# shininglegend/cs420-ray-tracer

Hardware: NVIDIA B200
Metric: Mrays/s (higher is better)
Workload: dtype f32 filter / f64 decide

## Files before the change

### cs420-ray-tracer_b200/csrc/kernels_fast.cuh

```cuda
#ifndef RT_KERNELS_FAST_CUH
#define RT_KERNELS_FAST_CUH

#include "bvh.cuh"
#include "exact_fp64.cuh"
#include "filter_math.cuh"
#include "rt_device.h"

namespace rtf {

using rtx::d3;

#ifndef RT_THREADS
#define RT_THREADS 256
#endif
constexpr int kThreads = RT_THREADS;
constexpr int kWarps = kThreads / 32;
constexpr unsigned kTwoMult = 1, kLpMult = 4;
constexpr int kWTileW = 16, kWTileH = 4;
constexpr int kGroupPairs = 4;
constexpr int kSmemHeader = 2048;
constexpr float kEps = 0.001f;
constexpr unsigned kSign = 0x80000000u;
constexpr unsigned kFull = 0xffffffffu;

struct __align__(16) RayRec {
  double ox, oy, oz, dx, dy, dz;
  unsigned pix;
  float wt;
  float ar, ag, ab;
  unsigned pad;
};

struct FastArgs {
  RtRenderArgs r;
  const unsigned char *tabs;
  int npairs, ngroups;
  int N, L;
  unsigned tstride, gmin_off, perm_off, inv_off, cullA_off, cullB_off;
  unsigned stage_bytes;
  float d64;
  float gS2;
  float g_dtmax;
  double c0[3];
  int wtiles_x, nwtiles;
  unsigned int *tile_counter;
  RayRec *q_out; unsigned int *q_out_count;
  RayRec *q_in; const unsigned int *q_in_count;
  unsigned int *chunk_counter;
  int level;
  int tables_in_smem;
  rtb::BvhView bvh;
  int nbig, big[8];
  unsigned two_mult, lp_mult;
  unsigned queue_cap;
  unsigned int *err;
};

struct Tab {
  const float4 *pairs;
  const float *gmin;
  const int *perm;
  const int *inv;
  const float4 *cullA;
  const float *cullB;
};

__device__ __forceinline__ unsigned fbits(float x) { return __float_as_uint(x); }
__device__ __forceinline__ float f_rd(double x) { return __double2float_rd(x); }
__device__ __forceinline__ float f_ru(double x) { return __double2float_ru(x); }
__device__ __forceinline__ d3 ldc3(const double *p) { return rtx::mk(p[0], p[1], p[2]); }
__device__ __forceinline__ double4 ld_sph64(const double4 *p) {
  const double2 *q = reinterpret_cast<const double2 *>(p);
  double2 a = __ldg(q), b = __ldg(q + 1);
  return make_double4(a.x, a.y, b.x, b.y);
}
__device__ __forceinline__ unsigned long long wsum(unsigned long long v) {
#pragma unroll
  for (int o = 16; o > 0; o >>= 1) v += __shfl_xor_sync(kFull, v, o);
// ... 29 lines not shown
  const float rdv = fmaxf(0.0f, __fmaf_rn(rz, vz, __fmaf_rn(ry, vy, __fmul_rn(rx, vx))));
  const float spec = __fmul_rn(0.5f, shin == 0.0f ? 1.0f : __powf(rdv, shin));
  sr = __fadd_rn(sr, __fmaf_rn(g_frame.light_col[l][0], spec, __fmul_rn(m.x, kd)));
  sg = __fadd_rn(sg, __fmaf_rn(g_frame.light_col[l][1], spec, __fmul_rn(m.y, kd)));
  sb = __fadd_rn(sb, __fmaf_rn(g_frame.light_col[l][2], spec, __fmul_rn(m.z, kd)));
}
__device__ __forceinline__ void write_final(const RtRenderArgs &r, unsigned pix, float cr, float cg, float cb) {
  size_t o = pix;
  if (r.out_remap) {
    const unsigned lr = pix / (unsigned)r.W, x = pix - lr * (unsigned)r.W;
    if (r.out_remap == 2) o = (size_t)rt_local_to_global_row(r.bands, (int)lr) * (size_t)r.W + x;
    else o = (size_t)(lr + (unsigned)r.out_y0) * (size_t)r.out_pitch + x + (unsigned)r.out_x0;
  }
  if (r.fb) { float *f = r.fb + o * 3; f[0] = cr; f[1] = cg; f[2] = cb; }
  else { unsigned char *q = r.rgb + o * 3; q[0] = (unsigned char)quant8(cr); q[1] = (unsigned char)quant8(cg); q[2] = (unsigned char)quant8(cb); }
}
__device__ __forceinline__ int warp_fetch(unsigned int *counter) {
  int v = 0;
  if ((threadIdx.x & 31) == 0) v = (int)atomicAdd(counter, 1u);
  return __shfl_sync(kFull, v, 0);
}

#define RT_PDL_SYNC() do { asm volatile("griddepcontrol.wait;" ::: "memory"); asm volatile("griddepcontrol.launch_dependents;" ::: "memory"); } while (0)

__device__ __forceinline__ void mbar_init(unsigned long long *bar, unsigned count) {
  unsigned a = (unsigned)__cvta_generic_to_shared(bar);
  asm volatile("mbarrier.init.shared::cta.b64 [%0], %1;" ::"r"(a), "r"(count));
  asm volatile("fence.mbarrier_init.release.cluster;" ::: "memory");
}
__device__ __forceinline__ void mbar_expect_tx(unsigned long long *bar, unsigned bytes) {
  unsigned a = (unsigned)__cvta_generic_to_shared(bar);
  asm volatile("mbarrier.arrive.expect_tx.shared::cta.b64 _, [%0], %1;" ::"r"(a), "r"(bytes) : "memory");
}
__device__ __forceinline__ void tma_bulk_g2s(void *dst, const void *src, unsigned bytes, unsigned long long *bar) {
  unsigned d = (unsigned)__cvta_generic_to_shared(dst), b = (unsigned)__cvta_generic_to_shared(bar);
  asm volatile("cp.async.bulk.shared::cluster.global.mbarrier::complete_tx::bytes [%0], [%1], %2, [%3];" ::"r"(d), "l"(src),
               "r"(bytes), "r"(b)
               : "memory");
}
__device__ __forceinline__ void mbar_wait(unsigned long long *bar, unsigned parity) {
  unsigned a = (unsigned)__cvta_generic_to_shared(bar);
  asm volatile(
      "{\n\t.reg .pred p;\n\t"
      "WAIT_%=:\n\t"
      "mbarrier.try_wait.parity.shared::cta.b64 p, [%0], %1;\n\t"
      "@p bra DONE_%=;\n\t"
// ... 1024 lines not shown
  }
  c.closest = c.hits = c.shadow = c.occluded = c.fp64 = c.violations = 0;
  n_fp64 = 0;
}

#ifndef RT_TAIL_THREADS
#define RT_TAIL_THREADS 128
#endif
#ifndef RT_TAIL_CTAS
#define RT_TAIL_CTAS 3
#endif
constexpr int kTailThreads = RT_TAIL_THREADS;
#ifdef RT_TAIL_TRACE
constexpr int kTraceWarps = 4096, kTraceLevels = 6, kTraceStamps = 12;
__device__ unsigned long long g_tail_trace[kTraceWarps * kTraceLevels * kTraceStamps];
#define RT_TT(k, extra) do { const unsigned long long x_ = (unsigned long long)(extra);    \
    if (tt_on && lane == 0 && level - a.level < kTraceLevels) g_tail_trace[(tt_warp * kTraceLevels + (level - a.level)) * kTraceStamps + (k)] = (unsigned long long)clock64() | (x_ << 48); } while (0)
#define RT_TG(k) do { if (tt_on && lane == 0 && level - a.level < kTraceLevels) { unsigned long long t_; asm volatile("mov.u64 %0, %globaltimer;" : "=l"(t_)); g_tail_trace[(tt_warp * kTraceLevels + (level - a.level)) * kTraceStamps + (k)] = t_; } } while (0)
#else
#define RT_TT(k, extra) do { } while (0)
#define RT_TG(k) do { } while (0)
#endif
template <bool kSmem, bool kBvh>
__global__ void __launch_bounds__(kTailThreads, RT_TAIL_CTAS) k_bounce(const FastArgs a) {
  extern __shared__ __align__(128) unsigned char smem[];
  const unsigned char *tabs = a.tabs + a.tstride;
  if (kSmem) { stage_tables(smem, tabs, a.stage_bytes); tabs = smem + kSmemHeader; }
  RT_PDL_SYNC();
  const unsigned nq = *a.q_in_count;
  if (nq == 0u) return;
  const WarpBuf wb = warp_buf(smem + kSmemHeader + ((a.stage_bytes + 127u) & ~127u));
  const float4 *gen = reinterpret_cast<const float4 *>(tabs + (size_t)a.L * a.tstride);
  const int lane = threadIdx.x & 31;
  const int depth = a.r.max_depth, L = a.L;
  Counters cnt = {0, 0, 0, 0, 0, 0};
  int n_fp64 = 0;
  unsigned c_cand = 0, c_walks = 0;
  RayRec *qin = a.q_in;
  const unsigned nwarps = gridDim.x * (unsigned)(kTailThreads / 32);
  const unsigned per = min(32u, max(4u, (nq + nwarps - 1u) / nwarps));
#ifdef RT_TAIL_TRACE
  const unsigned tt_warp = blockIdx.x * (unsigned)(kTailThreads / 32) + (threadIdx.x >> 5);
  bool tt_on = tt_warp < (unsigned)kTraceWarps;
#endif
  for (;;) {
    const int chunk = warp_fetch(a.chunk_counter);
    if ((unsigned)chunk * per >= nq) break;
// ... 171 lines not shown
          } else {
            final_ = true;
          }
        } else {
          add_scaled(cr, cg, cb, wt, sr, sg, sb);
          final_ = true;
        }
      }
      if (live[0] && final_) write_final(a.r, pix, cr, cg, cb);
      if (a.r.counters) {
        flush_counters(a, cnt, n_fp64, level);
        if (lane == 0 && c_walks) { atomicAdd(&a.r.counters[RT_CNT_CAND], (unsigned long long)c_cand); atomicAdd(&a.r.counters[RT_CNT_WALKS], (unsigned long long)c_walks); }
        c_cand = c_walks = 0;
      }
      RT_TT(5, __popc(__ballot_sync(kFull, cont))); RT_TG(7);
      live[0] = cont;
      if (!__any_sync(kFull, cont)) break;
    }
#ifdef RT_TAIL_TRACE
    tt_on = false;
#endif
  }
}

}
#endif
```

### cs420-ray-tracer_b200/csrc/kernels_wave.cuh

```cuda
#ifndef RT_KERNELS_WAVE_CUH
#define RT_KERNELS_WAVE_CUH

#include <type_traits>

#include "kernels_fast.cuh"

#ifndef RT_SHADOW_CTAS
#define RT_SHADOW_CTAS 2
#endif
#ifndef RT_CLOSEST_CTAS
#define RT_CLOSEST_CTAS 2
#endif
#ifndef RT_CLOSEST0_CTAS
#define RT_CLOSEST0_CTAS RT_CLOSEST_CTAS
#endif
namespace rtf {

struct __align__(16) HitRec {
  double px, py, pz;
  float nx, ny, nz;
  float vx, vy, vz;
  int idx;
  unsigned pix;
  unsigned src;
  float wt, ar, ag, ab;
  unsigned pad;
};
__device__ __forceinline__ double hit_d0x(const HitRec &h) { return __hiloint2double(__float_as_int(h.vz), __float_as_int(h.vy)); }
__device__ __forceinline__ double hit_d0y(const HitRec &h) { return __hiloint2double(__float_as_int(h.wt), (int)h.src); }
__device__ __forceinline__ double hit_d0z(const HitRec &h) { return __hiloint2double(__float_as_int(h.ag), __float_as_int(h.ar)); }
__device__ __forceinline__ unsigned hit_ray_rank(const HitRec &h) { return __float_as_uint(h.vx); }
static_assert(sizeof(HitRec) == 80, "hit record layout");

struct WaveArgs {
  FastArgs f;
  HitRec *hits; unsigned int *hit_count;
  unsigned int *hit_n;
  unsigned hit_cap;
  unsigned char *occ;
  int occ_bits;
  unsigned int *work_counter;
  Best *cand;
  unsigned int *work_counter2;
  unsigned int *tile_ray;
};

enum { CTL_TILE = 0, CTL_ERR = 5, CTL_TAIL = 8, CTL_SHADOW = 48, CTL_SHADE = 88, CTL_CLOSEST = 128, CTL_HITS = 168, CTL_RAYS = 208,
       CTL_WORDS = 256 };

__device__ __forceinline__ void hit_block(const WaveArgs &w, unsigned m0, unsigned m1, unsigned (&slot)[2]) {
  const int lane = threadIdx.x & 31;
  const unsigned n = (unsigned)(__popc(m0) + __popc(m1));
  unsigned base = 0;
  if (n != 0u) {
    if (lane == 0) {
      base = atomicAdd(w.hit_count, 64u);
      if (base + 64u > w.hit_cap) { atomicOr(w.f.err, (unsigned)RT_GUARD_HIT_BLOCKS); base = 0u; }
      w.hit_n[base >> 6] = n;
    }
    base = __shfl_sync(kFull, base, 0);
  }
  const unsigned lt = (1u << lane) - 1u;
  slot[0] = base + (unsigned)__popc(m0 & lt);
  slot[1] = base + (unsigned)__popc(m0) + (unsigned)__popc(m1 & lt);
}

__device__ __noinline__ void flush_counts(unsigned long long *counters, int level, unsigned closest, unsigned hits, unsigned shadow,
                                          unsigned occluded, unsigned fp64, unsigned violations, unsigned long long n_spheres,
                                          unsigned cand = 0, unsigned walks = 0, unsigned fallbacks = 0) {
  unsigned v[6] = {closest, hits, shadow, occluded, fp64, violations};
#pragma unroll
// ... 195 lines not shown
        c_closest++; c_fp64 += best[r].nfp64;
        if (best[r].idx >= 0) {
          HitRec *rec = w.hits + hslot[r];
          const int hi = finish_hit(a, best[r], src[r], pix[r], 0u, 1.0f, 0.f, 0.f, 0.f, rec, &c_viol, &c_fp64);
          hit = hi >= 0;
          if (!hit) { rec->idx = -1; rec->pix = pix[r]; }
          else cont[r] = depth > 1 && __ldg(&a.r.matx[hi]).y > 0.5f;
          if (a.r.hit_idx) a.r.hit_idx[(size_t)pix[r] * depth] = hit ? rec->idx : -1;
        } else if (a.r.hit_idx) a.r.hit_idx[(size_t)pix[r] * depth] = -1;
      }
      c_hits += hit;
      const Rgb skyc = sky_colour(dy[r]);
      const bool sky = live[r] && !hit;
      if (kBytes) {
        unsigned char *q = s_rgb + (((lane >> 4) * 2 + r) * kWTileW + (lane & 15)) * 3;
        q[0] = (unsigned char)quant8(sky ? skyc.r : 0.f);
        q[1] = (unsigned char)quant8(sky ? skyc.g : 0.f);
        q[2] = (unsigned char)quant8(sky ? skyc.b : 0.f);
      } else if (sky) {
        write_final(a.r, pix[r], skyc.r, skyc.g, skyc.b);
      }
    }
    {
      const unsigned k0 = __ballot_sync(kFull, cont[0]), k1 = __ballot_sync(kFull, cont[1]), lt = (1u << lane) - 1u;
      if (cont[0]) w.hits[hslot[0]].vx = __uint_as_float((unsigned)__popc(k0 & lt));
      if (cont[1]) w.hits[hslot[1]].vx = __uint_as_float((unsigned)(__popc(k0) + __popc(k1 & lt)));
      if (lane == 0 && tile_ok) w.tile_ray[tile] = (unsigned)(__popc(k0) + __popc(k1));
    }
    if (!kBytes) continue;
    __syncwarp();
    if (!tile_ok || deferred) { __syncwarp(); continue; }
    if (tx0 + kWTileW <= W && (W & 15) == 0) {
      if (lane < kWTileH * 3) {
        const int ty = lane / 3, seg = lane % 3;
        if (ty0 + ty < rows) {
          const size_t orow = kFrame ? (size_t)rt_local_to_global_row(a.r.bands, ty0 + ty) : (size_t)(ty0 + ty);
          *reinterpret_cast<uint4 *>(a.r.rgb + (orow * W + tx0) * 3 + seg * 16) =
              *reinterpret_cast<const uint4 *>(s_rgb + ty * kWTileW * 3 + seg * 16);
        }
      }
    } else {
#pragma unroll
      for (int r = 0; r < 2; r++) {
        if (x < W && lr[r] < rows) {
          const unsigned char *q = s_rgb + (((lane >> 4) * 2 + r) * kWTileW + (lane & 15)) * 3;
          unsigned char *o = a.r.rgb + (kFrame ? ((size_t)j[r] * W + x) : (size_t)pix[r]) * 3;
          o[0] = q[0]; o[1] = q[1]; o[2] = q[2];
        }
      }
    }
    __syncwarp();
  }
  if (a.r.counters) flush_counts(a.r.counters, 0, c_closest, c_hits, 0, 0, c_fp64, c_viol, (unsigned long long)a.N, c_cand, c_walks, c_fall);
}
template <int kMode>
__global__ void __launch_bounds__(kThreads, RT_CLOSEST0_CTAS) k_closest0(const WaveArgs w) {
  extern __shared__ __align__(128) unsigned char smem[];
  const FastArgs &a = w.f;
  const unsigned char *tabs = a.tabs;
  if (kMode == kTabSmem) { stage_tables(smem, a.tabs, a.stage_bytes); tabs = smem + kSmemHeader; }
  if (kMode == kTabStream) ring_init(smem);
  RT_PDL_SYNC();
  closest0_body<kMode>(w, smem, tabs, smem + kSmemHeader + (kMode == kTabBvh ? 0u : ((a.stage_bytes + 127u) & ~127u)));
}

template <bool kBvh, bool kCull = false>
__device__ __forceinline__ void closest1_body(const WaveArgs &w, const float4 *gen, unsigned char *smem) {
  const FastArgs &a = w.f;
  const unsigned nq = __ldcg(a.q_in_count);
  if (nq == 0u) return;
  const int lane = threadIdx.x & 31, depth = a.r.max_depth, level = a.level;
  unsigned c_closest = 0, c_hits = 0, c_fp64 = 0, c_viol = 0, c_cand = 0, c_walks = 0;
  const RayRec *qin = a.q_in;
  static_assert(kGenIds * 2 <= kWTileH * kWTileW * 3, "survivor list in the header's per-warp staging area");
  unsigned short *ids = kCull ? reinterpret_cast<unsigned short *>(smem + 64 + (threadIdx.x >> 5) * (kWTileH * kWTileW * 3)) : nullptr;
  const bool two = nq >= gridDim.x * (unsigned)kWarps * 64u * a.two_mult;
  const unsigned per = two ? 64u : 32u;
  for (;;) {
    const int chunk = warp_fetch(w.work_counter);
    if ((unsigned)chunk * per >= nq) break;
    bool live[2];
    unsigned qi[2], pix[2];
    float ox[2], oy[2], oz[2], dx[2], dy[2], dz[2], wt[2], cr[2], cg[2], cb[2];
#pragma unroll
    for (int r = 0; r < 2; r++) {
// ... 404 lines not shown
        }
      }
    }
  }
  if (a.r.counters) flush_counts(a.r.counters, 99, 0, 0, 0, 0, c_fp64, 0, 0);
}

#ifndef RT_SHADE_CTAS
#define RT_SHADE_CTAS 4
#endif
#ifndef RT_SHADE_UNROLL
#define RT_SHADE_UNROLL 1
#endif
constexpr int kShadeUnroll = RT_SHADE_UNROLL;
__device__ __forceinline__ void prefetch_l1(const void *p) { asm volatile("prefetch.global.L1 [%0];" ::"l"(p)); }
__device__ __forceinline__ void queue_put(const WaveArgs &w, unsigned pos, const RayRec &rec) {
  if (pos < w.f.queue_cap) w.f.q_out[pos] = rec;
  else atomicOr(w.f.err, (unsigned)RT_GUARD_RAY_QUEUE);
}

__device__ __forceinline__ void shade_body(const WaveArgs &w) {
  const FastArgs &a = w.f;
  const int level = a.level;
  const bool ordered = level == 0;
  const unsigned nh = __ldcg(w.hit_count);
  if (nh == 0u) return;
  const int lane = threadIdx.x & 31, L = a.L;
  unsigned c_shadow = 0, c_occ = 0;
  const unsigned G = gridDim.x * (unsigned)kWarps;
  if (ordered && tile_path(a)) {
    __shared__ __align__(16) unsigned char s_tiles[kWarps][kWTileH * kWTileW * 3];
    unsigned char *s_tile = s_tiles[threadIdx.x >> 5];
    const unsigned W = (unsigned)a.r.W, rows = (unsigned)a.r.bands.local_rows;
    const bool frame = a.r.out_remap == 2;
    for (unsigned blk = blockIdx.x * (unsigned)kWarps + (threadIdx.x >> 5); blk * 64u < nh; blk += G) {
      {
        const unsigned bn = blk + G;
        if (bn * 64u < nh) {
          const unsigned char *q = reinterpret_cast<const unsigned char *>(w.hits + bn * 64u) + lane * 128;
          prefetch_l1(q);
          if (lane < 8) prefetch_l1(q + 32 * 128);
          if (lane == 0) prefetch_l1(w.hit_n + bn);
          if (!w.occ_bits && lane < L) prefetch_l1(w.occ + (size_t)lane * w.hit_cap + bn * 64u);
        }
      }
      const unsigned nslots = w.hit_n[blk];
      const unsigned pix0 = w.hits[blk * 64u].pix;
      const unsigned ty0 = (pix0 / W) & ~(unsigned)(kWTileH - 1), tx0 = (pix0 % W) & ~(unsigned)(kWTileW - 1);
      const bool whole = ty0 + kWTileH <= rows;
      const unsigned qbase = w.tile_ray[(ty0 / kWTileH) * (unsigned)a.wtiles_x + tx0 / kWTileW];
      if (whole) {
#pragma unroll
        for (int r = 0; r < 2; r++) {
          const unsigned ly = (unsigned)(lane >> 4) * 2u + (unsigned)r, lx = (unsigned)lane & 15u;
          float fx, fz;
          const unsigned c = sky_rgb8(camera_dir_y(a, (int)(tx0 + lx), rt_local_to_global_row(a.r.bands, (int)(ty0 + ly)), fx, fz));
          unsigned char *q = s_tile + (ly * kWTileW + lx) * 3;
          q[0] = (unsigned char)c; q[1] = (unsigned char)(c >> 8); q[2] = (unsigned char)(c >> 16);
        }
      }
      __syncwarp();
#pragma unroll kShadeUnroll
      for (int half = 0; half < 2; half++) {
        const unsigned h = blk * 64u + (unsigned)half * 32u + lane;
        const bool live = (h & 63u) < nslots && w.hits[h].idx >= 0;
        bool cont = false;
        RayRec rec;
        unsigned rank = 0;
        if (live) {
          const HitRec hr = w.hits[h];
          unsigned long long occm = hr.pad;
          if (!w.occ_bits) {
            occm = 0ull;
            for (int l = 0; l < L; l++)
              if (w.occ[(size_t)l * w.hit_cap + h]) occm |= 1ull << l;
          }
          c_shadow += (unsigned)L; c_occ += (unsigned)__popcll(occm);
          const unsigned y = hr.pix / W, x = hr.pix - y * W;
          cont = shade_one(w, level, hr, occm, rec, whole ? s_tile + ((y - ty0) * kWTileW + (x - tx0)) * 3 : nullptr);
          rank = hit_ray_rank(hr);
        }
        if (cont) queue_put(w, qbase + rank, rec);
      }
      __syncwarp();
      if (whole && lane < kWTileH * 3) {
        const unsigned ty = (unsigned)lane / 3u, sg = (unsigned)lane % 3u;
        const size_t orow = frame ? (size_t)rt_local_to_global_row(a.r.bands, (int)(ty0 + ty)) : (size_t)(ty0 + ty);
        *reinterpret_cast<uint4 *>(a.r.rgb + (orow * W + tx0) * 3 + sg * 16) = *reinterpret_cast<const uint4 *>(s_tile + lane * 16);
      }
      __syncwarp();
    }
    if (a.r.counters) flush_counts(a.r.counters, 99, 0, 0, c_shadow, c_occ, 0, 0, (unsigned long long)a.N);
    return;
  }
  for (unsigned chunk = blockIdx.x * (unsigned)kWarps + (threadIdx.x >> 5); chunk * 32u < nh; chunk += G) {
    const unsigned h = chunk * 32u + lane;
    {
      const unsigned hn = h + G * 32u;
      if (hn < nh) {
        const unsigned char *q = reinterpret_cast<const unsigned char *>(w.hits + hn);
        prefetch_l1(q); prefetch_l1(q + 64);
        if (lane == 0) prefetch_l1(w.hit_n + (hn >> 6));
        if (!w.occ_bits && lane < L) prefetch_l1(w.occ + (size_t)lane * w.hit_cap + hn);
      }
    }
    const bool live = (h & 63u) < w.hit_n[h >> 6] && w.hits[h].idx >= 0;
    bool cont = false;
    RayRec rec;
    unsigned qpos = 0;
    if (live) {
      const HitRec hr = w.hits[h];
      unsigned long long occm = hr.pad;
      if (!w.occ_bits) {
        occm = 0ull;
        for (int l = 0; l < L; l++)
          if (w.occ[(size_t)l * w.hit_cap + h]) occm |= 1ull << l;
      }
      c_shadow += (unsigned)L; c_occ += (unsigned)__popcll(occm);
      cont = shade_one(w, level, hr, occm, rec);
      if (ordered && cont) {
        const unsigned y = hr.pix / (unsigned)a.r.W, x = hr.pix - y * (unsigned)a.r.W;
        qpos = w.tile_ray[(y / kWTileH) * (unsigned)a.wtiles_x + x / kWTileW] + hit_ray_rank(hr);
      }
    }
    if (ordered) { if (cont) queue_put(w, qpos, rec); }
    else queue_push(cont, rec, a.q_out, a.q_out_count, a.queue_cap, a.err);
  }
  if (a.r.counters) flush_counts(a.r.counters, 99, 0, 0, c_shadow, c_occ, 0, 0, (unsigned long long)a.N);
}
__global__ void __launch_bounds__(kThreads, RT_SHADE_CTAS) k_shade(const WaveArgs w) {
  RT_PDL_SYNC();
  shade_body(w);
}

}
#endif
```

### cs420-ray-tracer_b200/csrc/rt_kernels.cu

```cuda
#include "rt_kernels.h"

#include <algorithm>
#include <cmath>
#include <cstring>
#include <map>
#include <mutex>
#include <thread>
#include <tuple>
#include <vector>

__constant__ RtFrameConst g_frame;

#include "kernels_exact.cuh"
#include "kernels_fast.cuh"
#include "kernels_wave.cuh"

cudaError_t rtk_set_frame_const(const RtFrameConst *host_const, cudaStream_t stream) {
  return cudaMemcpyToSymbolAsync(g_frame, host_const, sizeof(RtFrameConst), 0, cudaMemcpyHostToDevice, stream);
}

int rtk_launch_exact(const RtRenderArgs &args, cudaStream_t stream) {
  dim3 block(128);
  dim3 grid((args.W + 31) / 32, (args.bands.local_rows + 3) / 4);
  rtk::k_exact<<<grid, block, 0, stream>>>(args);
// ... 538 lines not shown
    cudaFree(fs->tabs); fs->tabs = nullptr; fs->tabs_cap = 0;
    if (fs->h_stage) cudaFreeHost(fs->h_stage);
    fs->h_stage = nullptr; fs->h_stage_cap = 0;
    fs->sph64 = fs->mat = fs->matx = nullptr;
    cudaFree(fs->bvh_nodes_buf); cudaFree(fs->bvh_scratch); cudaFree(fs->raw_dev);
    fs->bvh_nodes_buf = fs->bvh_scratch = nullptr; fs->bvh_nodes_cap = fs->bvh_scratch_cap = 0;
    fs->raw_dev = nullptr; fs->raw_cap = 0;
  }
  fs->bvh_nodes = fs->bvh_leaves = nullptr; fs->bvh_nleaf = 0;
}

int rtk_fast_last_error(const RtFastWork *w, unsigned int *word) {
  *word = 0;
  if (!w->last_err) return 0;
  RTK_TRY(cudaMemcpy(word, w->last_err, sizeof(unsigned int), cudaMemcpyDeviceToHost));
  return 0;
}

void rtk_fast_free_work(RtFastWork *w) {
  cudaFree(w->queue[0]); cudaFree(w->queue[1]); cudaFree(w->ctl); cudaFree(w->hits); cudaFree(w->occ); cudaFree(w->hit_n); cudaFree(w->cand);
  w->last_err = nullptr;
  w->cand = nullptr; w->cand_cap = 0;
  cudaFree(w->tile_ray); w->tile_ray = nullptr; w->tile_cap = 0;
  if (w->h_fb) { cudaFreeHost(w->h_fb); cudaEventDestroy(w->fb_event); }
  w->h_fb = nullptr; w->fb_pending = 0; w->fb_levels = 0;
  w->queue[0] = w->queue[1] = nullptr; w->ctl = nullptr; w->hits = nullptr; w->occ = nullptr; w->hit_n = nullptr;
  w->queue_cap = w->hit_cap = w->occ_bytes = 0;
}

namespace {
template <typename K>
int resident_grid(K kernel, size_t smem, int num_sms, int threads = rtf::kThreads) {
  static std::mutex mu;
  static std::map<std::tuple<const void *, size_t, int>, int> cache;
  const auto key = std::make_tuple((const void *)kernel, smem, threads);
  std::lock_guard<std::mutex> lk(mu);
  auto it = cache.find(key);
  if (it == cache.end()) {
    int nb = 0;
    if (cudaOccupancyMaxActiveBlocksPerMultiprocessor(&nb, kernel, threads, smem) != cudaSuccess || nb < 1) nb = 1;
    it = cache.emplace(key, nb).first;
  }
  return std::max(1, it->second * num_sms);
}
thread_local cudaError_t g_launch_err = cudaSuccess;
template <typename K, typename A>
void launch(K kernel, int grid, int block, size_t smem, cudaStream_t stream, bool pdl, const A &arg) {
  cudaLaunchConfig_t cfg;
  memset(&cfg, 0, sizeof(cfg));
  cfg.gridDim = dim3((unsigned)grid); cfg.blockDim = dim3((unsigned)block); cfg.dynamicSmemBytes = smem; cfg.stream = stream;
  cudaLaunchAttribute at[1];
  at[0].id = cudaLaunchAttributeProgrammaticStreamSerialization;
  at[0].val.programmaticStreamSerializationAllowed = 1;
  cfg.attrs = at; cfg.numAttrs = pdl ? 1u : 0u;
  const cudaError_t e = cudaLaunchKernelEx(&cfg, kernel, arg);
  if (e != cudaSuccess && g_launch_err == cudaSuccess) g_launch_err = e;
}
inline size_t bvh_smem() { return rtf::kSmemHeader + rtf::kWarps * (size_t)(rtf::kWarpBufBytes + rtf::kBundleBufBytes); }
inline size_t staged_smem(size_t bytes) { return rtf::kSmemHeader + ((bytes + 127) & ~(size_t)127) + rtf::kWarps * (size_t)rtf::kWarpBufBytes; }
using rtf::CTL_TILE; using rtf::CTL_TAIL; using rtf::CTL_SHADOW; using rtf::CTL_SHADE; using rtf::CTL_CLOSEST; using rtf::CTL_HITS; using rtf::CTL_RAYS;
}

int rtk_launch_fast(const RtRenderArgs &args, const RtFastScene *fs, RtFastWork *w, cudaStream_t stream,
                    const cudaEvent_t *marks) {
  const size_t npix = (size_t)args.W * args.bands.local_rows;
  if (!w->ctl) RTK_TRY(cudaMalloc(&w->ctl, kCtlWords * sizeof(unsigned int)));
  const size_t hit_cap = ((size_t)((args.W + rtf::kWTileW - 1) / rtf::kWTileW) * ((args.bands.local_rows + rtf::kWTileH - 1) / rtf::kWTileH) + 2) * 64 +
                         (size_t)w->num_sms * 4 * rtf::kWarps * 128 * (size_t)rtf::kTwoMult;
  if (w->hit_cap < hit_cap || w->occ_bytes < hit_cap * (size_t)(fs->L > 0 ? fs->L : 1) || (args.max_depth > 1 && w->queue_cap < npix)) {
    RTK_TRY(cudaStreamSynchronize(stream));
    cudaFree(w->queue[0]); cudaFree(w->queue[1]); cudaFree(w->hits); cudaFree(w->occ); cudaFree(w->hit_n);
    w->queue[0] = w->queue[1] = nullptr; w->hits = nullptr; w->occ = nullptr; w->hit_n = nullptr; w->queue_cap = w->hit_cap = w->occ_bytes = 0;
    RTK_TRY(cudaMalloc(&w->hits, hit_cap * sizeof(rtf::HitRec)));
    RTK_TRY(cudaMalloc(&w->hit_n, (hit_cap / 64) * sizeof(unsigned int)));
    w->occ_bytes = hit_cap * (size_t)(fs->L > 0 ? fs->L : 1);
    RTK_TRY(cudaMalloc(&w->occ, w->occ_bytes));
    w->hit_cap = hit_cap;
    if (args.max_depth > 1) {
      RTK_TRY(cudaMalloc(&w->queue[0], npix * sizeof(rtf::RayRec)));
      RTK_TRY(cudaMalloc(&w->queue[1], npix * sizeof(rtf::RayRec)));
      w->queue_cap = npix;
    }

  }
  if (fs->bvh_nodes && args.max_depth > 1 && w->cand_cap < npix) {
    RTK_TRY(cudaStreamSynchronize(stream));
    cudaFree(w->cand); w->cand = nullptr; w->cand_cap = 0;
    RTK_TRY(cudaMalloc(&w->cand, npix * sizeof(rtf::Best)));
    w->cand_cap = npix;
  }
  const size_t ntiles = (size_t)((args.W + rtf::kWTileW - 1) / rtf::kWTileW) * ((args.bands.local_rows + rtf::kWTileH - 1) / rtf::kWTileH);
  const size_t tile_cap = (ntiles + 4 * rtf::kThreads - 1) / (4 * rtf::kThreads) * (4 * rtf::kThreads);
  if (w->tile_cap < tile_cap) {
    RTK_TRY(cudaStreamSynchronize(stream));
    cudaFree(w->tile_ray); w->tile_ray = nullptr; w->tile_cap = 0;
    RTK_TRY(cudaMalloc(&w->tile_ray, tile_cap * sizeof(unsigned int)));
    w->tile_cap = tile_cap;
  }
  RTK_TRY(cudaMemsetAsync(w->ctl, 0, kCtlWords * sizeof(unsigned int), stream));
  if (args.max_depth <= 0 && !args.fb && !args.out_remap) RTK_TRY(cudaMemsetAsync(args.rgb, 0, npix * 3, stream));

  g_launch_err = cudaSuccess;
  rtf::WaveArgs wa;
  memset(&wa, 0, sizeof(wa));
  rtf::FastArgs &a = wa.f;
  a.r = args;
  a.tabs = (const unsigned char *)fs->tabs;
  a.npairs = fs->npairs; a.ngroups = fs->ngroups; a.N = fs->N; a.L = fs->L;
  a.tstride = fs->tstride; a.gmin_off = fs->gmin_off; a.perm_off = fs->perm_off; a.inv_off = fs->inv_off;
  a.cullA_off = fs->cullA_off; a.cullB_off = fs->cullB_off;
  a.d64 = fs->d64; a.gS2 = fs->gS2; a.g_dtmax = fs->g_dtmax;
  for (int k = 0; k < 3; k++) a.c0[k] = fs->c0[k];
  a.wtiles_x = (args.W + rtf::kWTileW - 1) / rtf::kWTileW;
  a.nwtiles = a.wtiles_x * ((args.bands.local_rows + rtf::kWTileH - 1) / rtf::kWTileH);
  a.tile_counter = w->ctl + CTL_TILE;
  a.two_mult = rtf::kTwoMult; a.lp_mult = rtf::kLpMult;
  a.queue_cap = (unsigned)w->queue_cap; a.err = w->ctl + rtf::CTL_ERR;
  w->last_err = a.err;
  wa.hits = (rtf::HitRec *)w->hits; wa.hit_cap = (unsigned)hit_cap;
  wa.occ = w->occ; wa.hit_n = w->hit_n; wa.tile_ray = w->tile_ray;
  wa.occ_bits = fs->L <= 32;
  const size_t pairs_bytes = (size_t)fs->npairs * 32;
  const size_t light_bytes = (size_t)fs->L * fs->tstride;
  const bool cam_smem = fs->tstride <= kMaxSmemTables, light_smem = light_bytes <= kMaxSmemTables;
  const bool gen_smem = pairs_bytes <= kMaxSmemTables, in_smem = fs->bytes_bounce <= kMaxSmemTables;
  a.tables_in_smem = in_smem;
  const bool bvh = fs->bvh_nodes != nullptr;
  a.bvh.nodes = (const rtb::BvhNode *)fs->bvh_nodes;
  a.nbig = fs->nbig;
  for (int k = 0; k < 8; k++) a.big[k] = fs->big[k];
  const size_t stream_smem = rtf::kSmemHeader + 2 * (size_t)rtf::kTileBytes;
  int launches = 0;
  const bool pdl = marks == nullptr;

  int wave_levels = w->wave_levels > 0 ? w->wave_levels : (fs->bvh_nodes ? RT_MAX_LEVELS_INTERNAL : (npix >= 750000 ? 2 : 1));
  const unsigned long long fb_key = fs->generation * 1000003ull + (unsigned long long)npix * 131ull + (unsigned long long)args.max_depth;
  const bool fb_auto = w->wave_levels <= 0 && !fs->bvh_nodes && args.max_depth > 1;
  if (fb_auto) {
    if (!w->h_fb) {
      RTK_TRY(cudaHostAlloc(&w->h_fb, 34 * sizeof(unsigned int), cudaHostAllocDefault));
      RTK_TRY(cudaEventCreateWithFlags(&w->fb_event, cudaEventDisableTiming));
    }
    const cudaError_t fbq = w->fb_pending ? cudaEventQuery(w->fb_event) : cudaErrorNotReady;
    if (fbq != cudaSuccess) cudaGetLastError();
    if (w->fb_pending && fbq == cudaSuccess) {
      constexpr unsigned kWaveMinRays = 60000u;
      int lv = 1;
      while (lv < 33 && w->h_fb[lv] >= kWaveMinRays) lv++;
      w->fb_levels = lv; w->fb_key = w->fb_pending_key; w->fb_pending = 0;
    }
    if (w->fb_levels > 0 && w->fb_key == fb_key) wave_levels = w->fb_levels;
  }
  for (int level = 0; level < args.max_depth && level < wave_levels; level++) {
    a.level = level;
    wa.hit_count = w->ctl + CTL_HITS + level;
    if (level == 0) {
      a.stage_bytes = fs->tstride;
      const size_t smem = cam_smem ? staged_smem(a.stage_bytes) : stream_smem;
      const int cta_tiles = (a.nwtiles + rtf::kWarps - 1) / rtf::kWarps;
      if (bvh) { int g = resident_grid(rtf::k_closest0<rtf::kTabBvh>, bvh_smem(), w->num_sms); launch(rtf::k_closest0<rtf::kTabBvh>, g < cta_tiles ? g : cta_tiles, rtf::kThreads, bvh_smem(), stream, false, wa); }
      else if (cam_smem) { int g = resident_grid(rtf::k_closest0<rtf::kTabSmem>, smem, w->num_sms); launch(rtf::k_closest0<rtf::kTabSmem>, g < cta_tiles ? g : cta_tiles, rtf::kThreads, smem, stream, false, wa); }
      else { int g = resident_grid(rtf::k_closest0<rtf::kTabStream>, smem, w->num_sms); launch(rtf::k_closest0<rtf::kTabStream>, g < cta_tiles ? g : cta_tiles, rtf::kThreads, smem, stream, false, wa); }
    } else {
      a.q_in = (rtf::RayRec *)w->queue[(level - 1) & 1];
      a.q_in_count = w->ctl + CTL_RAYS + level;
      wa.work_counter = w->ctl + CTL_CLOSEST + level;
      a.stage_bytes = (unsigned)pairs_bytes;
      const size_t smem = rtf::kSmemHeader + (gen_smem ? a.stage_bytes : 0);
      if (bvh) {
        wa.cand = (rtf::Best *)w->cand;
        wa.work_counter2 = w->ctl + CTL_TAIL + level;
        launch(rtf::k_closest1_dyn, resident_grid(rtf::k_closest1_dyn, 0, w->num_sms), rtf::kThreads, 0, stream, pdl, wa);
        launches++;
        launch(rtf::k_closest1<false, true>, resident_grid(rtf::k_closest1<false, true>, rtf::kSmemHeader, w->num_sms), rtf::kThreads, rtf::kSmemHeader, stream, pdl, wa);
      }
      else if (gen_smem) launch(rtf::k_closest1<true, false>, resident_grid(rtf::k_closest1<true, false>, smem, w->num_sms), rtf::kThreads, smem, stream, pdl, wa);
      else launch(rtf::k_closest1<false, false>, resident_grid(rtf::k_closest1<false, false>, smem, w->num_sms), rtf::kThreads, smem, stream, pdl, wa);
    }
    launches++;
    if (level == 0 && marks) RTK_TRY(cudaEventRecord(marks[0], stream));
    a.q_out = (rtf::RayRec *)w->queue[level & 1];
    a.q_out_count = w->ctl + CTL_RAYS + level + 1;
    if (fs->L > 0 || level == 0) {
      wa.work_counter = w->ctl + CTL_SHADOW + level;
      a.stage_bytes = (unsigned)light_bytes;
      const size_t smem = light_smem ? staged_smem(a.stage_bytes) : stream_smem;
      if (bvh && level > 0) launch(rtf::k_shadow_dyn, resident_grid(rtf::k_shadow_dyn, 0, w->num_sms), rtf::kThreads, 0, stream, pdl, wa);
      else if (bvh) launch(rtf::k_shadow<rtf::kTabBvh>, resident_grid(rtf::k_shadow<rtf::kTabBvh>, bvh_smem(), w->num_sms), rtf::kThreads, bvh_smem(), stream, pdl, wa);
      else if (light_smem) launch(rtf::k_shadow<rtf::kTabSmem>, resident_grid(rtf::k_shadow<rtf::kTabSmem>, smem, w->num_sms), rtf::kThreads, smem, stream, pdl, wa);
      else launch(rtf::k_shadow<rtf::kTabStream>, resident_grid(rtf::k_shadow<rtf::kTabStream>, smem, w->num_sms), rtf::kThreads, smem, stream, pdl, wa);
      launches++;
    }
    if (level == 0 && marks) RTK_TRY(cudaEventRecord(marks[1], stream));
    wa.work_counter = w->ctl + CTL_SHADE + level;
    launch(rtf::k_shade, resident_grid(rtf::k_shade, 0, w->num_sms), rtf::kThreads, 0, stream, pdl, wa);
    launches++;
    if (level == 0 && marks) RTK_TRY(cudaEventRecord(marks[2], stream));
  }
  if (args.max_depth > wave_levels) {
    const int level = wave_levels;
    a.level = level;
    a.q_in = (rtf::RayRec *)w->queue[(level - 1) & 1];
    a.q_in_count = w->ctl + CTL_RAYS + level;
    a.q_out = (rtf::RayRec *)w->queue[level & 1];
    a.q_out_count = w->ctl + CTL_RAYS + level + 1;
    a.chunk_counter = w->ctl + CTL_TAIL + level;
    a.stage_bytes = (unsigned)fs->bytes_bounce;
    const size_t smem = in_smem ? staged_smem(fs->bytes_bounce) : rtf::kSmemHeader;
    if (bvh) launch(rtf::k_bounce<false, true>, resident_grid(rtf::k_bounce<false, true>, rtf::kSmemHeader, w->num_sms, rtf::kTailThreads), rtf::kTailThreads, rtf::kSmemHeader, stream, pdl, a);
    else if (in_smem) launch(rtf::k_bounce<true, false>, resident_grid(rtf::k_bounce<true, false>, smem, w->num_sms, rtf::kTailThreads), rtf::kTailThreads, smem, stream, pdl, a);
    else launch(rtf::k_bounce<false, false>, resident_grid(rtf::k_bounce<false, false>, smem, w->num_sms, rtf::kTailThreads), rtf::kTailThreads, smem, stream, pdl, a);
    launches++;
  }
  if (fb_auto && !w->fb_pending) {
    RTK_TRY(cudaMemcpyAsync(w->h_fb, w->ctl + CTL_RAYS, 34 * sizeof(unsigned int), cudaMemcpyDeviceToHost, stream));
    RTK_TRY(cudaEventRecord(w->fb_event, stream));
    w->fb_pending = 1; w->fb_pending_key = fb_key;
  }
  cudaError_t e = cudaGetLastError();
  if (g_launch_err != cudaSuccess) e = g_launch_err;
  return e == cudaSuccess ? launches : -(int)e;
}

__global__ void k_peer_signal(volatile unsigned int *flag, unsigned int value) {
  __threadfence_system();
  *flag = value;
  __threadfence_system();
}
__global__ void k_peer_wait(volatile unsigned int *flags, int n, unsigned int value, unsigned int *err) {
  const int k = threadIdx.x;
  if (k >= n) return;
  unsigned long long t0, t1;
  asm volatile("mov.u64 %0, %globaltimer;" : "=l"(t0));
  while ((int)(flags[k] - value) < 0) {
    asm volatile("mov.u64 %0, %globaltimer;" : "=l"(t1));
    if (t1 - t0 > 2000000000ULL) { atomicExch(err, 1u + (unsigned)k); break; }
    __nanosleep(200);
  }
  __threadfence_system();
}
int rtk_peer_signal(unsigned int *flag, unsigned int value, cudaStream_t stream) {
  k_peer_signal<<<1, 1, 0, stream>>>(flag, value);
  cudaError_t e = cudaGetLastError();
  return e == cudaSuccess ? 1 : -(int)e;
// ... 84 lines not shown
```

### cs420-ray-tracer_b200/csrc/rt_kernels.h

```cpp
#ifndef RT_KERNELS_H
#define RT_KERNELS_H

#include <cuda_runtime.h>

#include "rt_device.h"

cudaError_t rtk_set_frame_const(const RtFrameConst *host_const, cudaStream_t stream);

int rtk_launch_exact(const RtRenderArgs &args, cudaStream_t stream);

struct RtFastScene {
  int N, L, npairs, ngroups;
  void *tabs;
  size_t tabs_cap;
  void *sph64, *mat, *matx;
  void *h_stage; size_t h_stage_cap;
  void *raw_dev; size_t raw_cap;
  unsigned tstride;
  unsigned gmin_off, perm_off, inv_off, cullA_off, cullB_off;
  size_t bytes_primary;
  size_t bytes_bounce;
  float d64;
  float gS2;
  float g_dtmax;
  unsigned long long generation;
  double c0[3];
  void *bvh_nodes, *bvh_leaves;
  void *bvh_nodes_buf, *bvh_scratch;
  size_t bvh_nodes_cap, bvh_scratch_cap;
  int bvh_nleaf;
  int nbig, big[8];
  double bvh_build_ms;
  double sabs_scene;
  double delta64;
  int lookup_only, device_build;
  void *geo;
  void *cam_scratch; size_t cam_scratch_cap;
};
struct RtFastWork {
  int num_sms;
  int wave_levels;
  unsigned int *h_fb;
  cudaEvent_t fb_event;
  int fb_pending, fb_levels;
  unsigned long long fb_key, fb_pending_key;
  void *queue[2];
  size_t queue_cap;
  unsigned int *ctl;
  unsigned int *last_err;
  void *hits;
  unsigned int *hit_n;
  void *cand;
  size_t cand_cap;
  unsigned char *occ;
  size_t hit_cap, occ_bytes;
  unsigned int *tile_ray;
  size_t tile_cap;
};
int rtk_fast_init(int device);
int rtk_fast_build_scene(RtFastScene *fs, const double *spheres, int N, const RtFrameConst *frame, int accel, cudaStream_t stream);
void rtk_fast_free_scene(RtFastScene *fs, int release_tables);
double rtk_delta64(double sabs_scene, const double cam_pos[3]);
int rtk_fast_camera_table(RtFastScene *fs, const double cam_pos[3], cudaStream_t stream);
int rtk_camera_plane(double *su, int nu, double *sv, int nv, int m, int W, int H, double scale, cudaStream_t stream);
void rtk_fast_free_work(RtFastWork *w);
int rtk_fast_last_error(const RtFastWork *w, unsigned int *word);
int rtk_launch_fast(const RtRenderArgs &args, const RtFastScene *fs, RtFastWork *w, cudaStream_t stream,
                    const cudaEvent_t *marks);

int rtk_peer_signal(unsigned int *flag, unsigned int value, cudaStream_t stream);
int rtk_peer_wait(unsigned int *flags, int n, unsigned int value, unsigned int *err, cudaStream_t stream);
// ... 7 lines not shown
```

Baseline: 18630.

## Double-buffer control words, publish feedback via mapped memory, rank queue slots in shade

The per-frame cudaMemsetAsync of the control block is replaced by two alternating control sets, with the first closest kernel zeroing the next set on device. The feedback memcpy plus event is replaced by the last retiring warp of the final kernel writing counts and a sequence number into mapped host memory. Queue ranks are no longer stored in hit records; shade computes them with a warp ballot and a running offset. This removes a memset, a memcpy and an event from each frame, at the cost of a global retire atomic per warp and more complex cross-frame state.

```diff
diff --git a/cs420-ray-tracer_b200/csrc/kernels_fast.cuh b/cs420-ray-tracer_b200/csrc/kernels_fast.cuh
--- a/cs420-ray-tracer_b200/csrc/kernels_fast.cuh
+++ b/cs420-ray-tracer_b200/csrc/kernels_fast.cuh
@@ -30,6 +30,10 @@
   float ar, ag, ab;
   unsigned pad;
 };
+
+enum { CTL_TILE = 0, CTL_RETIRE = 1, CTL_ERR = 5, CTL_TAIL = 8, CTL_SHADOW = 48, CTL_SHADE = 88, CTL_CLOSEST = 128, CTL_HITS = 168,
+       CTL_RAYS = 208, CTL_WORDS = 256 };
+constexpr int kFbWords = 34;
 
 struct FastArgs {
   RtRenderArgs r;
@@ -54,6 +58,9 @@
   unsigned two_mult, lp_mult;
   unsigned queue_cap;
   unsigned int *err;
+  unsigned int *ctl;
+  unsigned int *fb_host;
+  unsigned fb_seq;
 };
 
 struct Tab {
@@ -129,6 +136,22 @@
 }
 
 #define RT_PDL_SYNC() do { asm volatile("griddepcontrol.wait;" ::: "memory"); asm volatile("griddepcontrol.launch_dependents;" ::: "memory"); } while (0)
+
+__device__ __noinline__ void publish_counts(unsigned int *ctl, unsigned int *fb_host, unsigned fb_seq) {
+  const int lane = threadIdx.x & 31;
+  __syncwarp();
+  unsigned last = 0;
+  if (lane == 0) {
+    __threadfence();
+    last = atomicAdd(ctl + CTL_RETIRE, 1u) == gridDim.x * (blockDim.x >> 5) - 1u;
+  }
+  if (!__shfl_sync(kFull, last, 0)) return;
+  __threadfence();
+  for (int k = lane; k < kFbWords; k += 32) fb_host[k] = __ldcg(ctl + CTL_RAYS + k);
+  __threadfence_system();
+  __syncwarp();
+  if (lane == 0) *reinterpret_cast<volatile unsigned *>(fb_host + kFbWords) = fb_seq;
+}
 
 __device__ __forceinline__ void mbar_init(unsigned long long *bar, unsigned count) {
   unsigned a = (unsigned)__cvta_generic_to_shared(bar);
@@ -1199,7 +1222,7 @@
 #define RT_TG(k) do { } while (0)
 #endif
 template <bool kSmem, bool kBvh>
-__global__ void __launch_bounds__(kTailThreads, RT_TAIL_CTAS) k_bounce(const FastArgs a) {
+__device__ __forceinline__ void bounce_body(const FastArgs &a) {
   extern __shared__ __align__(128) unsigned char smem[];
   const unsigned char *tabs = a.tabs + a.tstride;
   if (kSmem) { stage_tables(smem, tabs, a.stage_bytes); tabs = smem + kSmemHeader; }
@@ -1417,6 +1440,11 @@
 #endif
   }
 }
+template <bool kSmem, bool kBvh>
+__global__ void __launch_bounds__(kTailThreads, RT_TAIL_CTAS) k_bounce(const FastArgs a) {
+  bounce_body<kSmem, kBvh>(a);
+  if (a.fb_host) publish_counts(a.ctl, a.fb_host, a.fb_seq);
+}
 
 }
 #endif
diff --git a/cs420-ray-tracer_b200/csrc/kernels_wave.cuh b/cs420-ray-tracer_b200/csrc/kernels_wave.cuh
--- a/cs420-ray-tracer_b200/csrc/kernels_wave.cuh
+++ b/cs420-ray-tracer_b200/csrc/kernels_wave.cuh
@@ -29,7 +29,6 @@
 __device__ __forceinline__ double hit_d0x(const HitRec &h) { return __hiloint2double(__float_as_int(h.vz), __float_as_int(h.vy)); }
 __device__ __forceinline__ double hit_d0y(const HitRec &h) { return __hiloint2double(__float_as_int(h.wt), (int)h.src); }
 __device__ __forceinline__ double hit_d0z(const HitRec &h) { return __hiloint2double(__float_as_int(h.ag), __float_as_int(h.ar)); }
-__device__ __forceinline__ unsigned hit_ray_rank(const HitRec &h) { return __float_as_uint(h.vx); }
 static_assert(sizeof(HitRec) == 80, "hit record layout");
 
 struct WaveArgs {
@@ -43,10 +42,8 @@
   Best *cand;
   unsigned int *work_counter2;
   unsigned int *tile_ray;
+  unsigned int *ctl_next;
 };
-
-enum { CTL_TILE = 0, CTL_ERR = 5, CTL_TAIL = 8, CTL_SHADOW = 48, CTL_SHADE = 88, CTL_CLOSEST = 128, CTL_HITS = 168, CTL_RAYS = 208,
-       CTL_WORDS = 256 };
 
 __device__ __forceinline__ void hit_block(const WaveArgs &w, unsigned m0, unsigned m1, unsigned (&slot)[2]) {
   const int lane = threadIdx.x & 31;
@@ -288,9 +285,7 @@
       }
     }
     {
-      const unsigned k0 = __ballot_sync(kFull, cont[0]), k1 = __ballot_sync(kFull, cont[1]), lt = (1u << lane) - 1u;
-      if (cont[0]) w.hits[hslot[0]].vx = __uint_as_float((unsigned)__popc(k0 & lt));
-      if (cont[1]) w.hits[hslot[1]].vx = __uint_as_float((unsigned)(__popc(k0) + __popc(k1 & lt)));
+      const unsigned k0 = __ballot_sync(kFull, cont[0]), k1 = __ballot_sync(kFull, cont[1]);
       if (lane == 0 && tile_ok) w.tile_ray[tile] = (unsigned)(__popc(k0) + __popc(k1));
     }
     if (!kBytes) continue;
@@ -327,6 +322,8 @@
   if (kMode == kTabSmem) { stage_tables(smem, a.tabs, a.stage_bytes); tabs = smem + kSmemHeader; }
   if (kMode == kTabStream) ring_init(smem);
   RT_PDL_SYNC();
+  static_assert(CTL_WORDS == kThreads, "one control word per thread of CTA 0");
+  if (blockIdx.x == 0) w.ctl_next[threadIdx.x] = 0u;
   closest0_body<kMode>(w, smem, tabs, smem + kSmemHeader + (kMode == kTabBvh ? 0u : ((a.stage_bytes + 127u) & ~127u)));
 }
 
@@ -777,17 +774,17 @@
 __device__ __forceinline__ void shade_body(const WaveArgs &w) {
   const FastArgs &a = w.f;
   const int level = a.level;
-  const bool ordered = level == 0;
   const unsigned nh = __ldcg(w.hit_count);
   if (nh == 0u) return;
   const int lane = threadIdx.x & 31, L = a.L;
   unsigned c_shadow = 0, c_occ = 0;
   const unsigned G = gridDim.x * (unsigned)kWarps;
-  if (ordered && tile_path(a)) {
+  if (level == 0) {
     __shared__ __align__(16) unsigned char s_tiles[kWarps][kWTileH * kWTileW * 3];
     unsigned char *s_tile = s_tiles[threadIdx.x >> 5];
     const unsigned W = (unsigned)a.r.W, rows = (unsigned)a.r.bands.local_rows;
-    const bool frame = a.r.out_remap == 2;
+    const bool tiles = tile_path(a), frame = a.r.out_remap == 2;
+    const unsigned lt = (1u << lane) - 1u;
     for (unsigned blk = blockIdx.x * (unsigned)kWarps + (threadIdx.x >> 5); blk * 64u < nh; blk += G) {
       {
         const unsigned bn = blk + G;
@@ -802,7 +799,7 @@
       const unsigned nslots = w.hit_n[blk];
       const unsigned pix0 = w.hits[blk * 64u].pix;
       const unsigned ty0 = (pix0 / W) & ~(unsigned)(kWTileH - 1), tx0 = (pix0 % W) & ~(unsigned)(kWTileW - 1);
-      const bool whole = ty0 + kWTileH <= rows;
+      const bool whole = tiles && ty0 + kWTileH <= rows;
       const unsigned qbase = w.tile_ray[(ty0 / kWTileH) * (unsigned)a.wtiles_x + tx0 / kWTileW];
       if (whole) {
 #pragma unroll
@@ -815,13 +812,13 @@
         }
       }
       __syncwarp();
+      unsigned qpos = qbase;
 #pragma unroll kShadeUnroll
       for (int half = 0; half < 2; half++) {
         const unsigned h = blk * 64u + (unsigned)half * 32u + lane;
         const bool live = (h & 63u) < nslots && w.hits[h].idx >= 0;
         bool cont = false;
         RayRec rec;
-        unsigned rank = 0;
         if (live) {
           const HitRec hr = w.hits[h];
           unsigned long long occm = hr.pad;
@@ -833,9 +830,10 @@
           c_shadow += (unsigned)L; c_occ += (unsigned)__popcll(occm);
           const unsigned y = hr.pix / W, x = hr.pix - y * W;
           cont = shade_one(w, level, hr, occm, rec, whole ? s_tile + ((y - ty0) * kWTileW + (x - tx0)) * 3 : nullptr);
-          rank = hit_ray_rank(hr);
-        }
-        if (cont) queue_put(w, qbase + rank, rec);
+        }
+        const unsigned km = __ballot_sync(kFull, cont);
+        if (cont) queue_put(w, qpos + (unsigned)__popc(km & lt), rec);
+        qpos += (unsigned)__popc(km);
       }
       __syncwarp();
       if (whole && lane < kWTileH * 3) {
@@ -862,7 +860,6 @@
     const bool live = (h & 63u) < w.hit_n[h >> 6] && w.hits[h].idx >= 0;
     bool cont = false;
     RayRec rec;
-    unsigned qpos = 0;
     if (live) {
       const HitRec hr = w.hits[h];
       unsigned long long occm = hr.pad;
@@ -873,19 +870,15 @@
       }
       c_shadow += (unsigned)L; c_occ += (unsigned)__popcll(occm);
       cont = shade_one(w, level, hr, occm, rec);
-      if (ordered && cont) {
-        const unsigned y = hr.pix / (unsigned)a.r.W, x = hr.pix - y * (unsigned)a.r.W;
-        qpos = w.tile_ray[(y / kWTileH) * (unsigned)a.wtiles_x + x / kWTileW] + hit_ray_rank(hr);
-      }
-    }
-    if (ordered) { if (cont) queue_put(w, qpos, rec); }
-    else queue_push(cont, rec, a.q_out, a.q_out_count, a.queue_cap, a.err);
+    }
+    queue_push(cont, rec, a.q_out, a.q_out_count, a.queue_cap, a.err);
   }
   if (a.r.counters) flush_counts(a.r.counters, 99, 0, 0, c_shadow, c_occ, 0, 0, (unsigned long long)a.N);
 }
 __global__ void __launch_bounds__(kThreads, RT_SHADE_CTAS) k_shade(const WaveArgs w) {
   RT_PDL_SYNC();
   shade_body(w);
+  if (w.f.fb_host) publish_counts(w.f.ctl, w.f.fb_host, w.f.fb_seq);
 }
 
 }
diff --git a/cs420-ray-tracer_b200/csrc/rt_kernels.cu b/cs420-ray-tracer_b200/csrc/rt_kernels.cu
--- a/cs420-ray-tracer_b200/csrc/rt_kernels.cu
+++ b/cs420-ray-tracer_b200/csrc/rt_kernels.cu
@@ -584,9 +584,9 @@
   w->last_err = nullptr;
   w->cand = nullptr; w->cand_cap = 0;
   cudaFree(w->tile_ray); w->tile_ray = nullptr; w->tile_cap = 0;
-  if (w->h_fb) { cudaFreeHost(w->h_fb); cudaEventDestroy(w->fb_event); }
-  w->h_fb = nullptr; w->fb_pending = 0; w->fb_levels = 0;
-  w->queue[0] = w->queue[1] = nullptr; w->ctl = nullptr; w->hits = nullptr; w->occ = nullptr; w->hit_n = nullptr;
+  if (w->h_fb) cudaFreeHost(w->h_fb);
+  w->h_fb = w->d_fb = nullptr; w->fb_pending = 0; w->fb_levels = 0;
+  w->queue[0] = w->queue[1] = nullptr; w->ctl = nullptr; w->ctl_clean = 0; w->hits = nullptr; w->occ = nullptr; w->hit_n = nullptr;
   w->queue_cap = w->hit_cap = w->occ_bytes = 0;
 }
 
@@ -626,7 +626,7 @@
 int rtk_launch_fast(const RtRenderArgs &args, const RtFastScene *fs, RtFastWork *w, cudaStream_t stream,
                     const cudaEvent_t *marks) {
   const size_t npix = (size_t)args.W * args.bands.local_rows;
-  if (!w->ctl) RTK_TRY(cudaMalloc(&w->ctl, kCtlWords * sizeof(unsigned int)));
+  if (!w->ctl) RTK_TRY(cudaMalloc(&w->ctl, 2 * kCtlWords * sizeof(unsigned int)));
   const size_t hit_cap = ((size_t)((args.W + rtf::kWTileW - 1) / rtf::kWTileW) * ((args.bands.local_rows + rtf::kWTileH - 1) / rtf::kWTileH) + 2) * 64 +
                          (size_t)w->num_sms * 4 * rtf::kWarps * 128 * (size_t)rtf::kTwoMult;
   if (w->hit_cap < hit_cap || w->occ_bytes < hit_cap * (size_t)(fs->L > 0 ? fs->L : 1) || (args.max_depth > 1 && w->queue_cap < npix)) {
@@ -659,7 +659,12 @@
     RTK_TRY(cudaMalloc(&w->tile_ray, tile_cap * sizeof(unsigned int)));
     w->tile_cap = tile_cap;
   }
-  RTK_TRY(cudaMemsetAsync(w->ctl, 0, kCtlWords * sizeof(unsigned int), stream));
+  if (!w->ctl_clean) {
+    RTK_TRY(cudaMemsetAsync(w->ctl, 0, 2 * kCtlWords * sizeof(unsigned int), stream));
+    w->ctl_set = 0;
+  }
+  w->ctl_clean = 0;
+  unsigned int *const ctl = w->ctl + w->ctl_set * kCtlWords;
   if (args.max_depth <= 0 && !args.fb && !args.out_remap) RTK_TRY(cudaMemsetAsync(args.rgb, 0, npix * 3, stream));
 
   g_launch_err = cudaSuccess;
@@ -675,12 +680,14 @@
   for (int k = 0; k < 3; k++) a.c0[k] = fs->c0[k];
   a.wtiles_x = (args.W + rtf::kWTileW - 1) / rtf::kWTileW;
   a.nwtiles = a.wtiles_x * ((args.bands.local_rows + rtf::kWTileH - 1) / rtf::kWTileH);
-  a.tile_counter = w->ctl + CTL_TILE;
+  a.ctl = ctl;
+  a.tile_counter = ctl + CTL_TILE;
   a.two_mult = rtf::kTwoMult; a.lp_mult = rtf::kLpMult;
-  a.queue_cap = (unsigned)w->queue_cap; a.err = w->ctl + rtf::CTL_ERR;
+  a.queue_cap = (unsigned)w->queue_cap; a.err = ctl + rtf::CTL_ERR;
   w->last_err = a.err;
   wa.hits = (rtf::HitRec *)w->hits; wa.hit_cap = (unsigned)hit_cap;
   wa.occ = w->occ; wa.hit_n = w->hit_n; wa.tile_ray = w->tile_ray;
+  wa.ctl_next = w->ctl + (1 - w->ctl_set) * kCtlWords;
   wa.occ_bits = fs->L <= 32;
   const size_t pairs_bytes = (size_t)fs->npairs * 32;
   const size_t light_bytes = (size_t)fs->L * fs->tstride;
@@ -700,12 +707,11 @@
   const bool fb_auto = w->wave_levels <= 0 && !fs->bvh_nodes && args.max_depth > 1;
   if (fb_auto) {
     if (!w->h_fb) {
-      RTK_TRY(cudaHostAlloc(&w->h_fb, 34 * sizeof(unsigned int), cudaHostAllocDefault));
-      RTK_TRY(cudaEventCreateWithFlags(&w->fb_event, cudaEventDisableTiming));
-    }
-    const cudaError_t fbq = w->fb_pending ? cudaEventQuery(w->fb_event) : cudaErrorNotReady;
-    if (fbq != cudaSuccess) cudaGetLastError();
-    if (w->fb_pending && fbq == cudaSuccess) {
+      RTK_TRY(cudaHostAlloc(&w->h_fb, (rtf::kFbWords + 1) * sizeof(unsigned int), cudaHostAllocMapped));
+      RTK_TRY(cudaHostGetDevicePointer(&w->d_fb, w->h_fb, 0));
+      w->h_fb[rtf::kFbWords] = w->fb_seq;
+    }
+    if (w->fb_pending && __atomic_load_n(&w->h_fb[rtf::kFbWords], __ATOMIC_ACQUIRE) == w->fb_seq) {
       constexpr unsigned kWaveMinRays = 60000u;
       int lv = 1;
       while (lv < 33 && w->h_fb[lv] >= kWaveMinRays) lv++;
@@ -713,9 +719,12 @@
     }
     if (w->fb_levels > 0 && w->fb_key == fb_key) wave_levels = w->fb_levels;
   }
+  const bool publish = fb_auto && !w->fb_pending;
+  const bool tail = args.max_depth > wave_levels;
+  a.fb_seq = w->fb_seq + 1u;
   for (int level = 0; level < args.max_depth && level < wave_levels; level++) {
     a.level = level;
-    wa.hit_count = w->ctl + CTL_HITS + level;
+    wa.hit_count = ctl + CTL_HITS + level;
     if (level == 0) {
       a.stage_bytes = fs->tstride;
       const size_t smem = cam_smem ? staged_smem(a.stage_bytes) : stream_smem;
@@ -725,13 +734,13 @@
       else { int g = resident_grid(rtf::k_closest0<rtf::kTabStream>, smem, w->num_sms); launch(rtf::k_closest0<rtf::kTabStream>, g < cta_tiles ? g : cta_tiles, rtf::kThreads, smem, stream, false, wa); }
     } else {
       a.q_in = (rtf::RayRec *)w->queue[(level - 1) & 1];
-      a.q_in_count = w->ctl + CTL_RAYS + level;
-      wa.work_counter = w->ctl + CTL_CLOSEST + level;
+      a.q_in_count = ctl + CTL_RAYS + level;
+      wa.work_counter = ctl + CTL_CLOSEST + level;
       a.stage_bytes = (unsigned)pairs_bytes;
       const size_t smem = rtf::kSmemHeader + (gen_smem ? a.stage_bytes : 0);
       if (bvh) {
         wa.cand = (rtf::Best *)w->cand;
-        wa.work_counter2 = w->ctl + CTL_TAIL + level;
+        wa.work_counter2 = ctl + CTL_TAIL + level;
         launch(rtf::k_closest1_dyn, resident_grid(rtf::k_closest1_dyn, 0, w->num_sms), rtf::kThreads, 0, stream, pdl, wa);
         launches++;
         launch(rtf::k_closest1<false, true>, resident_grid(rtf::k_closest1<false, true>, rtf::kSmemHeader, w->num_sms), rtf::kThreads, rtf::kSmemHeader, stream, pdl, wa);
@@ -742,9 +751,9 @@
     launches++;
     if (level == 0 && marks) RTK_TRY(cudaEventRecord(marks[0], stream));
     a.q_out = (rtf::RayRec *)w->queue[level & 1];
-    a.q_out_count = w->ctl + CTL_RAYS + level + 1;
+    a.q_out_count = ctl + CTL_RAYS + level + 1;
     if (fs->L > 0 || level == 0) {
-      wa.work_counter = w->ctl + CTL_SHADOW + level;
+      wa.work_counter = ctl + CTL_SHADOW + level;
       a.stage_bytes = (unsigned)light_bytes;
       const size_t smem = light_smem ? staged_smem(a.stage_bytes) : stream_smem;
       if (bvh && level > 0) launch(rtf::k_shadow_dyn, resident_grid(rtf::k_shadow_dyn, 0, w->num_sms), rtf::kThreads, 0, stream, pdl, wa);
@@ -754,7 +763,8 @@
       launches++;
     }
     if (level == 0 && marks) RTK_TRY(cudaEventRecord(marks[1], stream));
-    wa.work_counter = w->ctl + CTL_SHADE + level;
+    wa.work_counter = ctl + CTL_SHADE + level;
+    a.fb_host = publish && !tail && level + 1 == args.max_depth ? w->d_fb : nullptr;
     launch(rtf::k_shade, resident_grid(rtf::k_shade, 0, w->num_sms), rtf::kThreads, 0, stream, pdl, wa);
     launches++;
     if (level == 0 && marks) RTK_TRY(cudaEventRecord(marks[2], stream));
@@ -763,25 +773,25 @@
     const int level = wave_levels;
     a.level = level;
     a.q_in = (rtf::RayRec *)w->queue[(level - 1) & 1];
-    a.q_in_count = w->ctl + CTL_RAYS + level;
+    a.q_in_count = ctl + CTL_RAYS + level;
     a.q_out = (rtf::RayRec *)w->queue[level & 1];
-    a.q_out_count = w->ctl + CTL_RAYS + level + 1;
-    a.chunk_counter = w->ctl + CTL_TAIL + level;
+    a.q_out_count = ctl + CTL_RAYS + level + 1;
+    a.chunk_counter = ctl + CTL_TAIL + level;
     a.stage_bytes = (unsigned)fs->bytes_bounce;
+    a.fb_host = publish ? w->d_fb : nullptr;
     const size_t smem = in_smem ? staged_smem(fs->bytes_bounce) : rtf::kSmemHeader;
     if (bvh) launch(rtf::k_bounce<false, true>, resident_grid(rtf::k_bounce<false, true>, rtf::kSmemHeader, w->num_sms, rtf::kTailThreads), rtf::kTailThreads, rtf::kSmemHeader, stream, pdl, a);
     else if (in_smem) launch(rtf::k_bounce<true, false>, resident_grid(rtf::k_bounce<true, false>, smem, w->num_sms, rtf::kTailThreads), rtf::kTailThreads, smem, stream, pdl, a);
     else launch(rtf::k_bounce<false, false>, resident_grid(rtf::k_bounce<false, false>, smem, w->num_sms, rtf::kTailThreads), rtf::kTailThreads, smem, stream, pdl, a);
     launches++;
   }
-  if (fb_auto && !w->fb_pending) {
-    RTK_TRY(cudaMemcpyAsync(w->h_fb, w->ctl + CTL_RAYS, 34 * sizeof(unsigned int), cudaMemcpyDeviceToHost, stream));
-    RTK_TRY(cudaEventRecord(w->fb_event, stream));
-    w->fb_pending = 1; w->fb_pending_key = fb_key;
-  }
   cudaError_t e = cudaGetLastError();
   if (g_launch_err != cudaSuccess) e = g_launch_err;
-  return e == cudaSuccess ? launches : -(int)e;
+  if (e != cudaSuccess) return -(int)e;
+  if (publish) { w->fb_seq++; w->fb_pending = 1; w->fb_pending_key = fb_key; }
+  if (launches > 0) w->ctl_set ^= 1;
+  w->ctl_clean = 1;
+  return launches;
 }
 
 __global__ void k_peer_signal(volatile unsigned int *flag, unsigned int value) {
diff --git a/cs420-ray-tracer_b200/csrc/rt_kernels.h b/cs420-ray-tracer_b200/csrc/rt_kernels.h
--- a/cs420-ray-tracer_b200/csrc/rt_kernels.h
+++ b/cs420-ray-tracer_b200/csrc/rt_kernels.h
@@ -41,12 +41,15 @@
   int num_sms;
   int wave_levels;
   unsigned int *h_fb;
-  cudaEvent_t fb_event;
+  unsigned int *d_fb;
+  unsigned fb_seq;
   int fb_pending, fb_levels;
   unsigned long long fb_key, fb_pending_key;
   void *queue[2];
   size_t queue_cap;
   unsigned int *ctl;
+  int ctl_set;
+  int ctl_clean;
   unsigned int *last_err;
   void *hits;
   unsigned int *hit_n;
```

Result: no change. 18710, median of 6 (+0.4%).
